# LordTARN1SHED/Image-Restoration-for-Road-Sign-Recognition-in-Autonomous-Driving

Hardware: AMD Instinct MI355X
Metric: images/sec ResUNet fwd+bwd (64x64 GTSRB batch) at 1/2/4/8 MI355X; PSNR parity (higher is better)
Workload: dtype bf16; 1 GPU; cfg3: ResUNet unified train step (dynamic distortion + ToTensor, fwd + L1 + 0.1*VGG16[:16] perceptual + bwd + AdamW), 14_train_unified_advanced.py; global_batch=512, per_gpu_batch=512, parallelism=dp1, hip_graph=True

## Files before the change

image-restoration-for-road-sign-recognition-in-autonomous-driving_amd/csrc/conv_in.hip:

```cpp
#include "common.h"

namespace {

template <typename T>
__global__ void conv_in_fwd_kernel(int n, int h, int w, int cin, int cout,
                                   const float *__restrict__ x, const float *__restrict__ wt,
                                   const float *__restrict__ b, int act, const float *alpha,
                                   T *__restrict__ y) {
  extern __shared__ __attribute__((aligned(16))) float sw[];
  const int kk = cin * 9;
  for (int i = threadIdx.x; i < kk * cout; i += blockDim.x) {
    const int co = i % cout, j = i / cout;
    sw[i] = wt[(long long)co * kk + j];
  }
  for (int i = threadIdx.x; i < cout; i += blockDim.x) sw[kk * cout + i] = b ? b[i] : 0.f;
  __syncthreads();
  const int G = cout / 4;
  const long long P = (long long)n * h * w;
  const float al = alpha ? alpha[0] : 0.f;
  for (long long id = blockIdx.x * (long long)blockDim.x + threadIdx.x; id < P * G;
       id += (long long)gridDim.x * blockDim.x) {
    const int g = (int)(id % G);
    const long long p = id / G;
    const int ww = (int)(p % w);
    const long long nh = p / w;
    const int hh = (int)(nh % h);
    const int nn = (int)(nh / h);
    f32x4 acc = *reinterpret_cast<const f32x4 *>(sw + kk * cout + g * 4);
    for (int ci = 0; ci < cin; ++ci) {
      const float *xp = x + ((long long)nn * cin + ci) * h * w;
#pragma unroll
      for (int t = 0; t < 9; ++t) {
        const int y2 = hh + t / 3 - 1, x2 = ww + t % 3 - 1;
        if (y2 < 0 || y2 >= h || x2 < 0 || x2 >= w) continue;
        const float v = xp[(long long)y2 * w + x2];
        acc += v * *reinterpret_cast<const f32x4 *>(sw + (ci * 9 + t) * cout + g * 4);
      }
    }
    if (act == 1) {
#pragma unroll
      for (int k = 0; k < 4; ++k) acc[k] = fmaxf(acc[k], 0.f);
    } else if (act == 2) {
#pragma unroll
      for (int k = 0; k < 4; ++k) acc[k] = acc[k] > 0.f ? acc[k] : al * acc[k];
    }
    store4<T>(y + p * cout + g * 4, acc);
  }
}

template <typename T>
__global__ void conv_in_wgrad_kernel(int n, int h, int w, int cin, int cout,
                                     const float *__restrict__ x, const T *__restrict__ dy,
                                     float *__restrict__ part, long long px_per_block) {
  __shared__ __attribute__((aligned(16))) float sdy[64][65];
  __shared__ __attribute__((aligned(16))) float spt[64][32];
  const int kk = cin * 9;
  const long long P = (long long)n * h * w;
  const long long pb = blockIdx.x * px_per_block;
  const long long pe = min(P, pb + px_per_block);
  const int co = threadIdx.x & 63, jg = threadIdx.x >> 6;
  double acc[8] = {0, 0, 0, 0, 0, 0, 0, 0};
  for (long long p0 = pb; p0 < pe; p0 += 64) {
    __syncthreads();
    for (int i = threadIdx.x; i < 64 * 64; i += blockDim.x) {
      const int r = i >> 6, c = i & 63;
      const long long p = p0 + r;
      sdy[r][c] = (p < pe && c < cout) ? Elt<T>::load(dy, p * cout + c) : 0.f;
    }
    for (int i = threadIdx.x; i < 64 * 32; i += blockDim.x) {
      const int r = i >> 5, j = i & 31;
      const long long p = p0 + r;
      float v = 0.f;
      if (p < pe) {
        if (j < kk) {
          const int ci = j / 9, t = j % 9;
          const int ww = (int)(p % w);
          const long long nh = p / w;
          const int hh = (int)(nh % h);
          const int nn = (int)(nh / h);
          const int y2 = hh + t / 3 - 1, x2 = ww + t % 3 - 1;
          if (y2 >= 0 && y2 < h && x2 >= 0 && x2 < w)
            v = x[(((long long)nn * cin + ci) * h + y2) * w + x2];
        } else if (j == kk) {
          v = 1.f;
        }
      }
      spt[r][j] = v;
    }
    __syncthreads();
    if (co < cout) {
      float st[8] = {0.f, 0.f, 0.f, 0.f, 0.f, 0.f, 0.f, 0.f};
#pragma unroll 4
      for (int r = 0; r < 64; ++r) {
        const float d = sdy[r][co];
        const f32x4 a0 = *reinterpret_cast<const f32x4 *>(&spt[r][jg * 8]);
        const f32x4 a1 = *reinterpret_cast<const f32x4 *>(&spt[r][jg * 8 + 4]);
#pragma unroll
        for (int k = 0; k < 4; ++k) { st[k] += d * a0[k]; st[4 + k] += d * a1[k]; }
      }
#pragma unroll
      for (int k = 0; k < 8; ++k) acc[k] += st[k];
    }
  }
  if (co < cout) {
#pragma unroll
    for (int k = 0; k < 8; ++k) part[((long long)blockIdx.x * cout + co) * 32 + jg * 8 + k] = (float)acc[k];
  }
}

constexpr int CIA_NPX = 64;
constexpr int CIA_ROW = CIA_NPX + 8;
constexpr int CIA_XROW = 32 + 8;
template <bool REC>
__global__ __launch_bounds__(256, REC ? 4 : 1) void conv_in_wgrad_act_kernel(
    int n, int h, int w, const float *__restrict__ x, const bf16_t *__restrict__ g,
    const bf16_t *__restrict__ t, int act, const float *__restrict__ alpha,
    float *__restrict__ part, long long ppb) {
  __shared__ __attribute__((aligned(16))) u16 gT[64 * CIA_ROW];
  __shared__ __attribute__((aligned(16))) u16 pT[32 * CIA_ROW];
  __shared__ __attribute__((aligned(16))) u16 pX[REC ? CIA_NPX * CIA_XROW : 8];
  __shared__ float red[256];
  const int tid = threadIdx.x, lane = tid & 63, wv = tid >> 6;
  const long long P = (long long)n * h * w, hw = (long long)h * w;
  const long long p0 = blockIdx.x * ppb, p1 = min(P, p0 + ppb);
  const float al = act == 2 ? alpha[0] : 0.f;
  float sa = 0.f;
  f32x4 acc[2] = {f32x4{0.f, 0.f, 0.f, 0.f}, f32x4{0.f, 0.f, 0.f, 0.f}};
  const int lc = tid & 7, lpp = tid >> 3;
  const int bn = lane & 15, bk = lane >> 4;
  const int sj = tid & 63, sg = tid >> 6;
  uint4 rg[2], rt[2] = {};
  float rp[8];
  auto load_step = [&](long long q0) __attribute__((always_inline)) {
#pragma unroll
    for (int j = 0; j < 2; ++j) {
      const long long p = q0 + 2 * lpp + j;
      const bool ok = p < p1;
      const long long e = (ok ? p : p0) * 64 + lc * 8;
      rg[j] = *reinterpret_cast<const uint4 *>(g + e);
      if constexpr (!REC) rt[j] = *reinterpret_cast<const uint4 *>(t + e);
      if (!ok) rg[j] = uint4{0u, 0u, 0u, 0u};
    }
    const long long p = q0 + sj;
    const bool live = p < p1;
    int img = 0, y = 0, xx0 = 0;
    if (live) {
      img = (int)(p / hw);
      const int rem = (int)(p - img * hw);
      y = rem / w;
      xx0 = rem - y * w;
    }
#pragma unroll
    for (int u = 0; u < 8; ++u) {
      const int r = sg + 4 * u;
      float val = 0.f;
      if (r < 27) {
        const int ci = r / 9, ky = (r % 9) / 3, kx = r % 3;
        const int yy = y + ky - 1, xx = xx0 + kx - 1;
        const bool ok = live && yy >= 0 && yy < h && xx >= 0 && xx < w;
        const float vv = x[ok ? (((long long)img * 3 + ci) * h + yy) * w + xx : 0];
        val = ok ? vv : 0.f;
      } else if (r == 27) {
        val = live ? 1.f : 0.f;
      }
      rp[u] = val;
    }
  };
  auto bf = [](uint32_t word, int hi) { return __uint_as_float(hi ? (word & 0xffff0000u) : (word << 16)); };
  bf16x8 fw = {};
  if constexpr (REC) fw = *reinterpret_cast<const bf16x8 *>(t + (wv * 16 + bn) * 32 + bk * 8);
  if (p0 < p1) load_step(p0);
  for (long long q0 = p0; q0 < p1; q0 += CIA_NPX) {
    if constexpr (REC) {
#pragma unroll
      for (int u = 0; u < 8; ++u) {
        const u16 pv = f32_to_bf16(rp[u]);
        pT[(sg + 4 * u) * CIA_ROW + sj] = pv;
        pX[sj * CIA_XROW + sg + 4 * u] = pv;
      }
      __syncthreads();
#pragma unroll
      for (int nb = 0; nb < 4; ++nb) {
        const bf16x8 fp = *reinterpret_cast<const bf16x8 *>(&pX[(nb * 16 + bn) * CIA_XROW + bk * 8]);
        const f32x4 tv = __builtin_amdgcn_mfma_f32_16x16x32_bf16(fw, fp, f32x4{0.f, 0.f, 0.f, 0.f}, 0, 0, 0);
#pragma unroll
        for (int i = 0; i < 4; ++i) gT[(wv * 16 + 4 * bk + i) * CIA_ROW + nb * 16 + bn] = f32_to_bf16(tv[i]);
      }
      __syncthreads();
    }
    u16 v[2][8];
    uint32_t tpair[8];
    if constexpr (REC) {
#pragma unroll
      for (int k = 0; k < 8; ++k)
        tpair[k] = *reinterpret_cast<const uint32_t *>(&gT[(lc * 8 + k) * CIA_ROW + 2 * lpp]);
    }
#pragma unroll
    for (int j = 0; j < 2; ++j) {
      const uint32_t gw[4] = {rg[j].x, rg[j].y, rg[j].z, rg[j].w};
      const uint32_t tw[4] = {rt[j].x, rt[j].y, rt[j].z, rt[j].w};
#pragma unroll
      for (int k = 0; k < 8; ++k) {
        const float gg = bf(gw[k >> 1], k & 1);
        const float tt = REC ? bf(tpair[k], j) : bf(tw[k >> 1], k & 1);
        const float gp = tt > 0.f ? gg : al * gg;
        sa += tt > 0.f ? 0.f : gg * tt;
        v[j][k] = f32_to_bf16(gp);
      }
    }
#pragma unroll
    for (int k = 0; k < 8; ++k)
      *reinterpret_cast<uint32_t *>(&gT[(lc * 8 + k) * CIA_ROW + 2 * lpp]) =
          (uint32_t)v[0][k] | ((uint32_t)v[1][k] << 16);
    if constexpr (!REC) {
#pragma unroll
      for (int u = 0; u < 8; ++u) pT[(sg + 4 * u) * CIA_ROW + sj] = f32_to_bf16(rp[u]);
    }
    __syncthreads();
    if (q0 + CIA_NPX < p1) load_step(q0 + CIA_NPX);
#pragma unroll
    for (int ks = 0; ks < 2; ++ks) {
      const int px = ks * 32 + bk * 8;
      const bf16x8 fa = *reinterpret_cast<const bf16x8 *>(&gT[(wv * 16 + bn) * CIA_ROW + px]);
#pragma unroll
      for (int nb = 0; nb < 2; ++nb) {
        const bf16x8 fb = *reinterpret_cast<const bf16x8 *>(&pT[(nb * 16 + bn) * CIA_ROW + px]);
        acc[nb] = __builtin_amdgcn_mfma_f32_16x16x32_bf16(fa, fb, acc[nb], 0, 0, 0);
      }
    }
    __syncthreads();
  }
  float *pw = part + (long long)blockIdx.x * (64 * 32 + 32);
#pragma unroll
  for (int nb = 0; nb < 2; ++nb)
#pragma unroll
    for (int i = 0; i < 4; ++i) pw[(wv * 16 + 4 * bk + i) * 32 + nb * 16 + bn] = acc[nb][i];
  red[tid] = sa;
  __syncthreads();
  for (int o = 128; o > 0; o >>= 1) {
    if (tid < o) red[tid] += red[tid + o];
    __syncthreads();
  }
  if (tid < 32) pw[64 * 32 + tid] = tid == 0 ? red[0] : 0.f;
}

__global__ void conv_in_wgrad_act_finalize(int chunks, const double *__restrict__ part, float *dw,
                                           float *db, float *dalpha) {
  const int i = blockIdx.x * blockDim.x + threadIdx.x;
  const int cols = 64 * 32 + 32;
  if (i > 64 * 32) return;
  double sv[1] = {0};
  rr_fixed_sum<1>(part + i, cols, chunks, sv);
  const double s = sv[0];
  if (i == 64 * 32) {
    if (dalpha) dalpha[0] = (float)s;
    return;
  }
  const int co = i / 32, j = i % 32;
  if (j < 27) dw[co * 27 + j] = (float)s;
  else if (j == 27 && db) db[co] = (float)s;
}

__global__ void conv_in_wgrad_finalize(int cout, int kk, int blocks, const double *__restrict__ part,
                                       float *dw, float *db) {
  const int i = blockIdx.x * blockDim.x + threadIdx.x;
  if (i >= cout * 32) return;
  const int co = i / 32, j = i % 32;
  if (j > kk) return;
  double sv[1] = {0};
  rr_fixed_sum<1>(part + i, (long long)cout * 32, blocks, sv);
  const double s = sv[0];
  if (j < kk) dw[(long long)co * kk + j] = (float)s;
  else if (db) db[co] = (float)s;
}

template <typename T>
__global__ void conv_in_dgrad_kernel(int n, int h, int w, int cin, int cout,
                                     const T *__restrict__ dy, const float *__restrict__ wt,
                                     float *__restrict__ dx, int accumulate) {
  extern __shared__ __attribute__((aligned(16))) float sw[];
  const int kk = cin * 9;
  for (int i = threadIdx.x; i < kk * cout; i += blockDim.x) {
    const int co = i % cout, j = i / cout;
    const int t = j / cin, ci = j % cin;
    sw[i] = wt[((long long)co * cin + ci) * 9 + t];
  }
  __syncthreads();
  const long long P = (long long)n * h * w;
  for (long long p = blockIdx.x * (long long)blockDim.x + threadIdx.x; p < P;
       p += (long long)gridDim.x * blockDim.x) {
    const int ww = (int)(p % w);
    const long long nh = p / w;
    const int hh = (int)(nh % h);
    const int nn = (int)(nh / h);
    float acc[4] = {0.f, 0.f, 0.f, 0.f};
    for (int t = 0; t < 9; ++t) {
      const int ky = t / 3, kx = t % 3;
      const int y2 = hh - ky + 1, x2 = ww - kx + 1;
      if (y2 < 0 || y2 >= h || x2 < 0 || x2 >= w) continue;
      const T *dp = dy + (((long long)nn * h + y2) * w + x2) * cout;
      for (int c = 0; c < cout; c += 4) {
        const f32x4 d = load4<T>(dp + c);
        for (int ci = 0; ci < cin && ci < 4; ++ci) {
          const f32x4 wv = *reinterpret_cast<const f32x4 *>(sw + (t * cin + ci) * cout + c);
          acc[ci] += d[0] * wv[0] + d[1] * wv[1] + d[2] * wv[2] + d[3] * wv[3];
        }
      }
    }
    for (int ci = 0; ci < cin && ci < 4; ++ci) {
      const long long o = (((long long)nn * cin + ci) * h + hh) * w + ww;
      dx[o] = accumulate ? dx[o] + acc[ci] : acc[ci];
    }
  }
}

template <typename T>
__global__ void im2col3_kernel(int n, int h, int w, int cin, int kpad, const float *__restrict__ x,
                               T *__restrict__ col) {
  const int G = kpad / 4;
  const long long total = (long long)n * h * w * G;
  const int kk = cin * 9;
  for (long long i = blockIdx.x * (long long)blockDim.x + threadIdx.x; i < total;
       i += (long long)gridDim.x * blockDim.x) {
    const int g = (int)(i % G);
    const long long p = i / G;
    const int ww = (int)(p % w);
    const long long nh = p / w;
    const int hh = (int)(nh % h);
    const int nn = (int)(nh / h);
    f32x4 v;
#pragma unroll
    for (int e = 0; e < 4; ++e) {
      const int j = g * 4 + e;
      float val = 0.f;
      if (j < kk) {
        const int ci = j / 9, t = j - (j / 9) * 9;
        const int y2 = hh + t / 3 - 1, x2 = ww + t % 3 - 1;
        if (y2 >= 0 && y2 < h && x2 >= 0 && x2 < w)
          val = x[(((long long)nn * cin + ci) * h + y2) * w + x2];
      } else if (j == kk) {
        val = 1.f;
      }
      v[e] = val;
    }
    store4<T>(col + p * kpad + g * 4, v);
  }
}

__global__ __launch_bounds__(256) void conv_in_mfma_kernel(int n, int h, int w,
                                                           const float *__restrict__ x,
                                                           const bf16_t *__restrict__ wp, int act,
                                                           const float *__restrict__ alpha,
                                                           bf16_t *__restrict__ y_pre,
                                                           bf16_t *__restrict__ y_act) {
  constexpr int SR = 68;
  __shared__ __attribute__((aligned(16))) float stg[4][32 * SR];
  const int lane = threadIdx.x & 63, wv = threadIdx.x >> 6;
  const long long hw = (long long)h * w;
  const long long P = (long long)n * hw;
  const long long p0 = ((long long)blockIdx.x * 4 + wv) * 64;
  if (p0 >= P) return;
  const int fr = lane & 15, q = lane >> 4;
  bf16x8 fa[4];
#pragma unroll
  for (int mi = 0; mi < 4; ++mi)
    fa[mi] = *reinterpret_cast<const bf16x8 *>(wp + (mi * 16 + fr) * 32 + q * 8);
  const int hwi = h * w;
  int kofs[8], kdy[8], kdx[8];
  bool ktap[8], kone[8];
#pragma unroll
  for (int j = 0; j < 8; ++j) {
    const int k = q * 8 + j;
    const int ci = k / 9, t = k - (k / 9) * 9;
    kdy[j] = t / 3 - 1;
    kdx[j] = t % 3 - 1;
    kofs[j] = ci * hwi + kdy[j] * w + kdx[j];
    ktap[j] = k < 27;
    kone[j] = k == 27;
  }
  const int Pi = (int)P;
  const __amdgpu_buffer_rsrc_t xr = __builtin_amdgcn_make_buffer_rsrc(
      const_cast<float *>(x), 0, (int)(3 * P * 4), 0x00020000);
  const int pw0 = (int)p0;
  f32x4 acc[4][4];
#pragma unroll
  for (int ni = 0; ni < 4; ++ni) {
    const int p = pw0 + ni * 16 + fr;
    const bool live = p < Pi;
    const int pc = live ? p : 0;
    const int nn = pc / hwi, rem = pc - (pc / hwi) * hwi;
    const int yy = rem / w, xx = rem - (rem / w) * w;
    const int base = nn * 3 * hwi + rem;
    bf16x8 fb;
#pragma unroll
    for (int j = 0; j < 8; ++j) {
      const int y2 = yy + kdy[j], x2 = xx + kdx[j];
      const bool ok = ktap[j] && live && (unsigned)y2 < (unsigned)h && (unsigned)x2 < (unsigned)w;
      const float v = __builtin_bit_cast(float, __builtin_amdgcn_raw_buffer_load_b32(
          xr, ok ? (base + kofs[j]) * 4 : 0xffffffff, 0, 0));
      fb[j] = (__bf16)(v + (kone[j] ? 1.f : 0.f));
    }
#pragma unroll
    for (int mi = 0; mi < 4; ++mi)
      acc[mi][ni] = __builtin_amdgcn_mfma_f32_16x16x32_bf16(fa[mi], fb, f32x4{0.f, 0.f, 0.f, 0.f},
                                                           0, 0, 0);
  }
  float *sw = stg[wv];
  const float slope = act == 2 ? alpha[0] : (act == 1 ? 0.f : 1.f);
  const int rows = (int)min(64LL, P - p0);
#pragma unroll
  for (int half = 0; half < 2; ++half) {
    if (half) asm volatile("s_waitcnt lgkmcnt(0)" ::: "memory");
#pragma unroll
    for (int mi = 0; mi < 4; ++mi)
#pragma unroll
      for (int nj = 0; nj < 2; ++nj)
        *reinterpret_cast<f32x4 *>(sw + (nj * 16 + fr) * SR + mi * 16 + q * 4) = acc[mi][half * 2 + nj];
    asm volatile("s_waitcnt lgkmcnt(0)" ::: "memory");
#pragma unroll
    for (int i = 0; i < 4; ++i) {
      const int rl = i * 8 + (lane >> 3), c8 = (lane & 7) * 8;
      const int r = half * 32 + rl;
      if (r < rows) {
        const long long p = p0 + r;
        const f32x4 v0 = *reinterpret_cast<const f32x4 *>(sw + rl * SR + c8);
        const f32x4 v1 = *reinterpret_cast<const f32x4 *>(sw + rl * SR + c8 + 4);
        if (y_pre) store8<bf16_t>(y_pre + p * 64 + c8, v0, v1);
        if (y_act) {
          f32x4 a0, a1;
#pragma unroll
          for (int k = 0; k < 4; ++k) {
            a0[k] = v0[k] > 0.f ? v0[k] : slope * v0[k];
            a1[k] = v1[k] > 0.f ? v1[k] : slope * v1[k];
          }
          store8<bf16_t>(y_act + p * 64 + c8, a0, a1);
        }
      }
    }
  }
}

}

extern "C" int rr_im2col3(int dtype, int n, int h, int w, int cin, int kpad, const float *x,
                          void *col, rr_stream stream) {
  if (!x || !col || cin <= 0 || kpad % 4 || kpad < 9 * cin + 1) return RR_EINVAL;
  const long long total = (long long)n * h * w * (kpad / 4);
  dim3 g(rr_grid_cap((total + 255) / 256, 8192)), b(256);
  hipStream_t st = (hipStream_t)stream;
  return rr_dispatch_elt(dtype, [&](auto tag) {
    using T = typename decltype(tag)::type;
    hipLaunchKernelGGL(im2col3_kernel<T>, g, b, 0, st, n, h, w, cin, kpad, x, (T *)col);
    RR_CHECK_LAUNCH();
    return RR_OK;
  });
}

extern "C" int rr_conv_in_fwd(int dtype, int n, int h, int w, int cin, int cout, const float *x,
                              const float *wt, const float *b, int act, const float *alpha,
                              void *y, rr_stream stream) {
  if (!x || !wt || !y || n <= 0 || h <= 0 || w <= 0 || cin <= 0 || cin > 4 || cout % 4 ||
      cout > 128 || (act == 2 && !alpha))
    return RR_EINVAL;
  const long long work = (long long)n * h * w * (cout / 4);
  const size_t shm = ((size_t)cin * 9 * cout + cout) * sizeof(float);
  dim3 g(rr_grid_cap((work + 255) / 256, 8192)), bl(256);
  hipStream_t st = (hipStream_t)stream;
  return rr_dispatch_elt(dtype, [&](auto tag) {
    using T = typename decltype(tag)::type;
    hipLaunchKernelGGL(conv_in_fwd_kernel<T>, g, bl, shm, st, n, h, w, cin, cout, x, wt, b, act,
                       alpha, (T *)y);
    RR_CHECK_LAUNCH();
    return RR_OK;
  });
}

int rr_colreduce_misc(const float *in, int rows, int cols, double *out, hipStream_t st);
static int conv_in_wgrad_blocks(int n, int h, int w) {
  const long long P = (long long)n * h * w;
  long long b = (P + 2047) / 2048;
  if (b > 1024) b = 1024;
  return (int)(b < 1 ? 1 : b);
}

extern "C" size_t rr_conv_in_wgrad_workspace(int n, int h, int w, int cin, int cout) {
  (void)cin;
  const int blocks = conv_in_wgrad_blocks(n, h, w);
  return (size_t)blocks * cout * 32 * sizeof(float) + rr_colreduce_bytes(blocks, cout * 32);
}

extern "C" int rr_conv_in_wgrad(int dtype, int n, int h, int w, int cin, int cout, const float *x,
                                const void *dy, float *dw, float *db, void *ws, size_t ws_bytes,
                                rr_stream stream) {
  if (!x || !dy || !dw || cin * 9 >= 32 || cout > 64 || cout <= 0) return RR_EINVAL;
  const int blocks = conv_in_wgrad_blocks(n, h, w);
  const size_t pbytes = (size_t)blocks * cout * 32 * sizeof(float);
  if (!ws || ws_bytes < pbytes + rr_colreduce_bytes(blocks, cout * 32)) return RR_EWORKSPACE;
  const long long P = (long long)n * h * w;
  long long ppb = (P + blocks - 1) / blocks;
  hipStream_t st = (hipStream_t)stream;
  const int rc = rr_dispatch_elt(dtype, [&](auto tag) {
    using T = typename decltype(tag)::type;
    hipLaunchKernelGGL(conv_in_wgrad_kernel<T>, dim3(blocks), dim3(256), 0, st, n, h, w, cin, cout,
                       x, (const T *)dy, (float *)ws, ppb);
    RR_CHECK_LAUNCH();
    return RR_OK;
  });
  if (rc != RR_OK) return rc;
  double *red = (double *)((char *)ws + pbytes);
  const int chunks = rr_colreduce_misc((const float *)ws, blocks, cout * 32, red, st);
  if (chunks < 0) return RR_ELAUNCH;
  hipLaunchKernelGGL(conv_in_wgrad_finalize, dim3((cout * 32 + 255) / 256), dim3(256), 0, st, cout,
                     cin * 9, chunks, (const double *)red, dw, db);
  RR_CHECK_LAUNCH();
  return RR_OK;
}

static int conv_in_act_blocks(long long P) {
  long long b = (P + 511) / 512;
  if (b > 2048) b = 2048;
  return (int)(b < 1 ? 1 : b);
}

extern "C" size_t rr_conv_in_wgrad_act_workspace(int n, int h, int w) {
  const int blocks = conv_in_act_blocks((long long)n * h * w);
  return (size_t)blocks * (64 * 32 + 32) * sizeof(float) + rr_colreduce_bytes(blocks, 64 * 32 + 32);
}

static int conv_in_wgrad_act(bool rec, int n, int h, int w, const float *x, const void *dy,
                             const void *t_pre, int act, const float *alpha, float *dw, float *db,
                             float *dalpha, void *ws, size_t ws_bytes, rr_stream stream) {
  if (!x || !dy || !t_pre || !dw || n <= 0 || h <= 0 || w <= 0) return RR_EINVAL;
  if (act < 1 || act > 2 || (act == 2 && !alpha)) return RR_EINVAL;
// ... 67 lines not shown
```

image-restoration-for-road-sign-recognition-in-autonomous-driving_amd/csrc/conv_out.hip:

```cpp
#include "common.h"

namespace {

template <typename T>
__global__ void conv_out_fwd_kernel(int n, int h, int w, int cin, int cout, const T *__restrict__ x,
                                    const float *__restrict__ wt, const float *__restrict__ b,
                                    float *__restrict__ y) {
  extern __shared__ __attribute__((aligned(16))) float sw[];
  for (int i = threadIdx.x; i < cin * cout; i += blockDim.x) sw[i] = wt[i];
  __syncthreads();
  const long long P = (long long)n * h * w;
  const long long hw = (long long)h * w;
  for (long long p = blockIdx.x * (long long)blockDim.x + threadIdx.x; p < P;
       p += (long long)gridDim.x * blockDim.x) {
    float acc[4] = {0.f, 0.f, 0.f, 0.f};
    const T *xp = x + p * cin;
    for (int c = 0; c < cin; c += 4) {
      const f32x4 v = load4<T>(xp + c);
      for (int co = 0; co < cout && co < 4; ++co) {
        const f32x4 wv = *reinterpret_cast<const f32x4 *>(sw + co * cin + c);
        acc[co] += v[0] * wv[0] + v[1] * wv[1] + v[2] * wv[2] + v[3] * wv[3];
      }
    }
    const long long nn = p / hw, r = p % hw;
    for (int co = 0; co < cout && co < 4; ++co)
      y[(nn * cout + co) * hw + r] = acc[co] + (b ? b[co] : 0.f);
  }
}

template <typename T>
__global__ void conv_out_bwd_kernel(int n, int h, int w, int cin, int cout,
                                    const float *__restrict__ dy, const T *__restrict__ x,
                                    const float *__restrict__ wt, T *__restrict__ dx, int mask_relu,
                                    float *__restrict__ part, long long px_per_block) {
  __shared__ float red[4][64][4];
  __shared__ float redb[4][4];
  const int ci = threadIdx.x & 63, row = threadIdx.x >> 6;
  const long long hw = (long long)h * w;
  const long long P = (long long)n * hw;
  const long long pb = blockIdx.x * px_per_block;
  const long long pe = min(P, pb + px_per_block);
  float wv[4] = {0.f, 0.f, 0.f, 0.f};
  for (int co = 0; co < cout; ++co) wv[co] = ci < cin ? wt[co * cin + ci] : 0.f;
  float sw[4] = {0.f, 0.f, 0.f, 0.f}, sb[4] = {0.f, 0.f, 0.f, 0.f};
  for (long long p = pb + row; p < pe; p += 4) {
    const long long nn = p / hw, r = p - nn * hw;
    float d[4] = {0.f, 0.f, 0.f, 0.f};
    for (int co = 0; co < cout; ++co) d[co] = dy[(nn * cout + co) * hw + r];
    if (ci < cin) {
      const float xv = Elt<T>::load(x, p * cin + ci);
      float g = 0.f;
      for (int co = 0; co < cout; ++co) {
        g += d[co] * wv[co];
        sw[co] += d[co] * xv;
      }
      if (mask_relu && !(xv > 0.f)) g = 0.f;
      if (dx) Elt<T>::store(dx, p * cin + ci, g);
    }
    for (int co = 0; co < cout; ++co) sb[co] += d[co];
  }
  for (int co = 0; co < 4; ++co) red[row][ci][co] = sw[co];
  if (ci == 0)
    for (int co = 0; co < 4; ++co) redb[row][co] = sb[co];
  __syncthreads();
  if (row == 0 && ci < cin)
    for (int co = 0; co < cout; ++co)
      part[((long long)blockIdx.x * (cout + 1) + co) * cin + ci] =
          red[0][ci][co] + red[1][ci][co] + red[2][ci][co] + red[3][ci][co];
  if (threadIdx.x < cout) {
    const int co = threadIdx.x;
    part[((long long)blockIdx.x * (cout + 1) + cout) * cin + co] =
        redb[0][co] + redb[1][co] + redb[2][co] + redb[3][co];
  }
}

template <typename T, int COUT>
__global__ __launch_bounds__(256) void conv_out_bwd64_kernel(
    int n, int h, int w, const float *__restrict__ dy, const T *__restrict__ x,
    const float *__restrict__ wt, T *__restrict__ dx, int mask_relu, float *__restrict__ part,
    long long px_per_block) {
  constexpr int CIN = 64;
  __shared__ float red[4][COUT + 1][CIN];
  const int cg = threadIdx.x & 7, pl = threadIdx.x >> 3;
  const long long hw = (long long)h * w;
  const long long P = (long long)n * hw;
  const long long pb = blockIdx.x * px_per_block;
  const long long pe = min(P, pb + px_per_block);
  float wv[COUT][8];
#pragma unroll
  for (int co = 0; co < COUT; ++co)
#pragma unroll
    for (int j = 0; j < 8; ++j) wv[co][j] = wt[co * CIN + cg * 8 + j];
  float sw[COUT][8], sb[COUT];
#pragma unroll
  for (int co = 0; co < COUT; ++co) {
    sb[co] = 0.f;
#pragma unroll
    for (int j = 0; j < 8; ++j) sw[co][j] = 0.f;
  }
  auto one = [&](long long p) __attribute__((always_inline)) {
    const long long nn = p / hw, r = p - nn * hw;
    float d[COUT];
#pragma unroll
    for (int co = 0; co < COUT; ++co) d[co] = dy[(nn * COUT + co) * hw + r];
    const T *xp = x + p * CIN + cg * 8;
    const f32x4 x0 = load4<T>(xp), x1 = load4<T>(xp + 4);
    const float xv[8] = {x0[0], x0[1], x0[2], x0[3], x1[0], x1[1], x1[2], x1[3]};
    float g[8];
#pragma unroll
    for (int j = 0; j < 8; ++j) {
      float t = 0.f;
#pragma unroll
      for (int co = 0; co < COUT; ++co) {
        t += d[co] * wv[co][j];
        sw[co][j] += d[co] * xv[j];
      }
      g[j] = (mask_relu && !(xv[j] > 0.f)) ? 0.f : t;
    }
#pragma unroll
    for (int co = 0; co < COUT; ++co) sb[co] += d[co];
    if (dx) store8<T>(dx + p * CIN + cg * 8, f32x4{g[0], g[1], g[2], g[3]}, f32x4{g[4], g[5], g[6], g[7]});
  };
  long long p = pb + pl;
  for (; p + 32 < pe; p += 64) {
    one(p);
    one(p + 32);
  }
  if (p < pe) one(p);
#pragma unroll
  for (int co = 0; co < COUT; ++co) {
#pragma unroll
    for (int j = 0; j < 8; ++j) {
      float v = sw[co][j];
      v += __shfl_xor(v, 8, 64);
      v += __shfl_xor(v, 16, 64);
      v += __shfl_xor(v, 32, 64);
      sw[co][j] = v;
    }
    float v = sb[co];
    v += __shfl_xor(v, 8, 64);
    v += __shfl_xor(v, 16, 64);
    v += __shfl_xor(v, 32, 64);
    sb[co] = v;
  }
  const int wv_ = threadIdx.x >> 6, lane = threadIdx.x & 63;
  if (lane < 8) {
#pragma unroll
    for (int co = 0; co < COUT; ++co) {
#pragma unroll
      for (int j = 0; j < 8; ++j) red[wv_][co][cg * 8 + j] = sw[co][j];
      if (cg == 0) red[wv_][COUT][co] = sb[co];
    }
  }
  __syncthreads();
  for (int i = threadIdx.x; i < COUT * CIN + COUT; i += 256) {
    const int co = i / CIN, ci = i - co * CIN;
    part[(long long)blockIdx.x * (COUT + 1) * CIN + i] =
        red[0][co][ci] + red[1][co][ci] + red[2][co][ci] + red[3][co][ci];
  }
}

template <typename T, int COUT, bool REC = false>
__global__ __launch_bounds__(256) void conv_out_bwd64_bnred_kernel(
    int n, int h, int w, const float *__restrict__ dy, const T *__restrict__ x,
    const float *__restrict__ wt, const T *__restrict__ t0, const float *__restrict__ mean0,
    const float *__restrict__ inv0, const T *__restrict__ t1, const float *__restrict__ mean1,
    const float *__restrict__ inv1, float *__restrict__ part, float *__restrict__ bnpart,
    long long px_per_block, const float *__restrict__ aff_s = nullptr,
    const float *__restrict__ aff_b = nullptr) {
  constexpr int CIN = 64;
  __shared__ float red[4][COUT + 1][CIN];
  __shared__ float bred[4][CIN][3];
  const int cg = threadIdx.x & 7, pl = threadIdx.x >> 3;
  const long long hw = (long long)h * w;
  const long long P = (long long)n * hw;
  const long long pb = blockIdx.x * px_per_block;
  const long long pe = min(P, pb + px_per_block);
  float wv[COUT][8], m0[8], i0[8], m1[8], i1[8];
#pragma unroll
  for (int j = 0; j < 8; ++j) {
#pragma unroll
    for (int co = 0; co < COUT; ++co) wv[co][j] = wt[co * CIN + cg * 8 + j];
    m0[j] = mean0[cg * 8 + j]; i0[j] = inv0[cg * 8 + j];
    m1[j] = mean1[cg * 8 + j]; i1[j] = inv1[cg * 8 + j];
  }
  __shared__ __attribute__((aligned(16))) float faff[REC ? 4 * CIN : 4];
  if constexpr (REC) {
    faff[threadIdx.x] = threadIdx.x < 2 * CIN ? aff_s[threadIdx.x] : aff_b[threadIdx.x - 2 * CIN];
    __syncthreads();
  }
  float sw[COUT][8], sb[COUT], bs[3][8];
#pragma unroll
  for (int co = 0; co < COUT; ++co) {
    sb[co] = 0.f;
#pragma unroll
    for (int j = 0; j < 8; ++j) sw[co][j] = 0.f;
  }
#pragma unroll
  for (int j = 0; j < 8; ++j) { bs[0][j] = 0.f; bs[1][j] = 0.f; bs[2][j] = 0.f; }
  auto one = [&](long long p) __attribute__((always_inline)) {
    const long long nn = p / hw, r = p - nn * hw;
    float d[COUT];
#pragma unroll
    for (int co = 0; co < COUT; ++co) d[co] = dy[(nn * COUT + co) * hw + r];
    const long long e = p * CIN + cg * 8;
    f32x4 x0, x1, a0, a1, b0, b1;
    load8<T>(t0 + e, a0, a1);
    load8<T>(t1 + e, b0, b1);
    if constexpr (REC) {
      int o = cg * 8;
      asm volatile("" : "+v"(o));
      const f32x4 *fa = reinterpret_cast<const f32x4 *>(faff + o);
      f32x4 v0 = a0 * fa[0] + fa[32], v1 = a1 * fa[1] + fa[33];
      f32x4 q0 = b0 * fa[16] + fa[48], q1 = b1 * fa[17] + fa[49];
      v0 += q0;
      v1 += q1;
#pragma unroll
      for (int k = 0; k < 4; ++k) {
        x0[k] = Elt<T>::round(fmaxf(v0[k], 0.f));
        x1[k] = Elt<T>::round(fmaxf(v1[k], 0.f));
      }
    } else {
      load8<T>(x + e, x0, x1);
    }
    const float xv[8] = {x0[0], x0[1], x0[2], x0[3], x1[0], x1[1], x1[2], x1[3]};
    const float ta[8] = {a0[0], a0[1], a0[2], a0[3], a1[0], a1[1], a1[2], a1[3]};
    const float tb[8] = {b0[0], b0[1], b0[2], b0[3], b1[0], b1[1], b1[2], b1[3]};
#pragma unroll
    for (int j = 0; j < 8; ++j) {
      float t = 0.f;
#pragma unroll
      for (int co = 0; co < COUT; ++co) {
        t += d[co] * wv[co][j];
        sw[co][j] += d[co] * xv[j];
      }
      const float gm = xv[j] > 0.f ? Elt<T>::round(t) : 0.f;
      bs[0][j] += gm;
      bs[1][j] += gm * ((ta[j] - m0[j]) * i0[j]);
      bs[2][j] += gm * ((tb[j] - m1[j]) * i1[j]);
    }
#pragma unroll
    for (int co = 0; co < COUT; ++co) sb[co] += d[co];
  };
  long long p = pb + pl;
  for (; p + 32 < pe; p += 64) {
    one(p);
    one(p + 32);
  }
  if (p < pe) one(p);
  auto lanes8 = [](float v) __attribute__((always_inline)) {
    v += __shfl_xor(v, 8, 64);
    v += __shfl_xor(v, 16, 64);
    v += __shfl_xor(v, 32, 64);
    return v;
  };
#pragma unroll
  for (int co = 0; co < COUT; ++co) {
#pragma unroll
    for (int j = 0; j < 8; ++j) sw[co][j] = lanes8(sw[co][j]);
    sb[co] = lanes8(sb[co]);
  }
#pragma unroll
  for (int k = 0; k < 3; ++k)
#pragma unroll
    for (int j = 0; j < 8; ++j) bs[k][j] = lanes8(bs[k][j]);
  const int wv_ = threadIdx.x >> 6, lane = threadIdx.x & 63;
  if (lane < 8) {
#pragma unroll
    for (int co = 0; co < COUT; ++co) {
#pragma unroll
      for (int j = 0; j < 8; ++j) red[wv_][co][cg * 8 + j] = sw[co][j];
      if (cg == 0) red[wv_][COUT][co] = sb[co];
    }
#pragma unroll
    for (int j = 0; j < 8; ++j)
#pragma unroll
      for (int k = 0; k < 3; ++k) bred[wv_][cg * 8 + j][k] = bs[k][j];
  }
  __syncthreads();
  for (int i = threadIdx.x; i < COUT * CIN + COUT; i += 256) {
    const int co = i / CIN, ci = i - co * CIN;
    part[(long long)blockIdx.x * (COUT + 1) * CIN + i] =
        red[0][co][ci] + red[1][co][ci] + red[2][co][ci] + red[3][co][ci];
  }
  if (threadIdx.x < CIN * 3) {
    const int c = threadIdx.x / 3, k = threadIdx.x - c * 3;
    bnpart[(long long)blockIdx.x * CIN * 3 + threadIdx.x] =
        bred[0][c][k] + bred[1][c][k] + bred[2][c][k] + bred[3][c][k];
  }
}

constexpr int TCO_D = 2;
__global__ __launch_bounds__(256) void tail_conv_out_kernel(
    int P, int hw, int cout, const bf16_t *__restrict__ x, const float *__restrict__ scale,
    const float *__restrict__ shift, const bf16_t *__restrict__ res, const float *__restrict__ rs,
    const float *__restrict__ rb, const bf16_t *__restrict__ wp, const float *__restrict__ bias,
    bf16_t *__restrict__ y, float *__restrict__ out) {
  const int lane = threadIdx.x & 63;
  const int wv = __builtin_amdgcn_readfirstlane(threadIdx.x >> 6);
  const int fr = lane & 15, fq = lane >> 4;
  const int nblk = (P + 15) >> 4;
  const int gw = blockIdx.x * 4 + wv, NWT = gridDim.x * 4;
  bf16x8 wr[2];
  f32x4 s[2][2], b[2][2], qs[2][2], qb[2][2];
#pragma unroll
  for (int kb = 0; kb < 2; ++kb) {
    bf16x8 v = {};
    if (fr < cout) v = *reinterpret_cast<const bf16x8 *>(wp + fr * 64 + kb * 32 + fq * 8);
    wr[kb] = v;
#pragma unroll
    for (int hf = 0; hf < 2; ++hf) {
      const int c = kb * 32 + fq * 8 + 4 * hf;
      s[kb][hf] = *reinterpret_cast<const f32x4 *>(scale + c);
      b[kb][hf] = *reinterpret_cast<const f32x4 *>(shift + c);
      qs[kb][hf] = *reinterpret_cast<const f32x4 *>(rs + c);
      qb[kb][hf] = *reinterpret_cast<const f32x4 *>(rb + c);
    }
  }
  float bv[4];
#pragma unroll
  for (int j = 0; j < 4; ++j) bv[j] = j < cout ? bias[j] : 0.f;
  struct Blk {
    uint4 t[2], r[2];
  };
  auto load_blk = [&](int bi, Blk &bk) __attribute__((always_inline)) {
    const int p = min(bi * 16 + fr, P - 1);
    const long long e = (long long)p * 64 + fq * 8;
#pragma unroll
    for (int kb = 0; kb < 2; ++kb) {
      bk.t[kb] = *reinterpret_cast<const uint4 *>(x + e + kb * 32);
      bk.r[kb] = *reinterpret_cast<const uint4 *>(res + e + kb * 32);
    }
  };
  auto unpack = [](uint4 r, f32x4 &lo, f32x4 &hi) __attribute__((always_inline)) {
    lo[0] = __uint_as_float(r.x << 16); lo[1] = __uint_as_float(r.x & 0xffff0000u);
    lo[2] = __uint_as_float(r.y << 16); lo[3] = __uint_as_float(r.y & 0xffff0000u);
    hi[0] = __uint_as_float(r.z << 16); hi[1] = __uint_as_float(r.z & 0xffff0000u);
    hi[2] = __uint_as_float(r.w << 16); hi[3] = __uint_as_float(r.w & 0xffff0000u);
  };
  auto run = [&](const Blk &bk, int bi) __attribute__((always_inline)) {
    const int p = bi * 16 + fr;
    const bool live = p < P;
    f32x4 acc = f32x4{0.f, 0.f, 0.f, 0.f};
#pragma unroll
    for (int kb = 0; kb < 2; ++kb) {
      f32x4 v0, v1, q0, q1;
      unpack(bk.t[kb], v0, v1);
      unpack(bk.r[kb], q0, q1);
      v0 = v0 * s[kb][0] + b[kb][0];
      v1 = v1 * s[kb][1] + b[kb][1];
      q0 = q0 * qs[kb][0] + qb[kb][0];
      q1 = q1 * qs[kb][1] + qb[kb][1];
      v0 += q0;
      v1 += q1;
#pragma unroll
      for (int k = 0; k < 4; ++k) { v0[k] = fmaxf(v0[k], 0.f); v1[k] = fmaxf(v1[k], 0.f); }
      u16x8 r;
      r[0] = f32_to_bf16(v0[0]); r[1] = f32_to_bf16(v0[1]); r[2] = f32_to_bf16(v0[2]); r[3] = f32_to_bf16(v0[3]);
      r[4] = f32_to_bf16(v1[0]); r[5] = f32_to_bf16(v1[1]); r[6] = f32_to_bf16(v1[2]); r[7] = f32_to_bf16(v1[3]);
      if (y && live) *reinterpret_cast<u16x8 *>(y + (long long)p * 64 + kb * 32 + fq * 8) = r;
      acc = __builtin_amdgcn_mfma_f32_16x16x32_bf16(wr[kb], __builtin_bit_cast(bf16x8, r), acc, 0, 0, 0);
    }
    if (live && fq == 0) {
      const int n = p / hw, rem = p - n * hw;
#pragma unroll
      for (int j = 0; j < 4; ++j)
        if (j < cout) out[((long long)n * cout + j) * hw + rem] = acc[j] + bv[j];
    }
  };
  for (int b0 = gw; b0 < nblk; b0 += TCO_D * NWT) {
    Blk bk[TCO_D];
#pragma unroll
    for (int j = 0; j < TCO_D; ++j) load_blk(min(b0 + j * NWT, nblk - 1), bk[j]);
#pragma unroll
    for (int j = 0; j < TCO_D; ++j)
      if (b0 + j * NWT < nblk) run(bk[j], b0 + j * NWT);
  }
}

__global__ void conv_out_bwd_finalize(int cin, int cout, int blocks, const double *__restrict__ part,
                                      float *dw, float *db) {
  const int i = blockIdx.x * blockDim.x + threadIdx.x;
  if (i >= cout * cin + cout) return;
  double s = 0;
  if (i < cout * cin) {
    double sv[1] = {0};
    rr_fixed_sum<1>(part + i, (long long)(cout + 1) * cin, blocks, sv);
    s = sv[0];
    if (dw) dw[i] = (float)s;
  } else {
    const int co = i - cout * cin;
    double sv[1] = {0};
    rr_fixed_sum<1>(part + (long long)cout * cin + co, (long long)(cout + 1) * cin, blocks, sv);
    s = sv[0];
    if (db) db[co] = (float)s;
  }
}

}

extern "C" int rr_conv_out_fwd(int dtype, int n, int h, int w, int cin, int cout, const void *x,
                               const float *wt, const float *b, float *y, rr_stream stream) {
  if (!x || !wt || !y || cout > 4 || cout <= 0 || cin % 4) return RR_EINVAL;
  const long long P = (long long)n * h * w;
  dim3 g(rr_grid_cap((P + 255) / 256, 8192)), bl(256);
  const size_t shm = (size_t)cin * cout * sizeof(float);
  hipStream_t st = (hipStream_t)stream;
  return rr_dispatch_elt(dtype, [&](auto tag) {
    using T = typename decltype(tag)::type;
    hipLaunchKernelGGL(conv_out_fwd_kernel<T>, g, bl, shm, st, n, h, w, cin, cout, (const T *)x, wt,
                       b, y);
    RR_CHECK_LAUNCH();
    return RR_OK;
  });
}

int rr_colreduce_misc(const float *in, int rows, int cols, double *out, hipStream_t st);
static int conv_out_blocks(int n, int h, int w) {
  const long long P = (long long)n * h * w;
  long long b = (P + 1023) / 1024;
  if (b > 2048) b = 2048;
  return (int)(b < 1 ? 1 : b);
}

extern "C" size_t rr_conv_out_bwd_workspace(int n, int h, int w, int cin, int cout) {
  const int blocks = conv_out_blocks(n, h, w);
  return (size_t)blocks * (cout + 1) * cin * sizeof(float) +
         rr_colreduce_bytes(blocks, (cout + 1) * cin);
}

extern "C" int rr_conv_out_bwd(int dtype, int n, int h, int w, int cin, int cout, const float *dy,
                               const void *x, const float *wt, void *dx, int mask_relu, float *dw,
                               float *db, void *ws, size_t ws_bytes, rr_stream stream) {
  if (!dy || !x || !wt || cout > 4 || cout <= 0 || cin > 64 || cin < cout) return RR_EINVAL;
  const int blocks = conv_out_blocks(n, h, w);
  const size_t pbytes = (size_t)blocks * (cout + 1) * cin * sizeof(float);
  if (!ws || ws_bytes < pbytes + rr_colreduce_bytes(blocks, (cout + 1) * cin)) return RR_EWORKSPACE;
  const long long P = (long long)n * h * w;
  const long long ppb = (P + blocks - 1) / blocks;
  hipStream_t st = (hipStream_t)stream;
  const int rc = cin == 64 && cout == 3 ? rr_dispatch_elt(dtype, [&](auto tag) {
    using T = typename decltype(tag)::type;
    hipLaunchKernelGGL((conv_out_bwd64_kernel<T, 3>), dim3(blocks), dim3(256), 0, st, n, h, w, dy,
                       (const T *)x, wt, (T *)dx, mask_relu, (float *)ws, ppb);
    RR_CHECK_LAUNCH();
    return RR_OK;
  }) : rr_dispatch_elt(dtype, [&](auto tag) {
    using T = typename decltype(tag)::type;
    hipLaunchKernelGGL(conv_out_bwd_kernel<T>, dim3(blocks), dim3(256), 0, st, n, h, w, cin, cout, dy,
                       (const T *)x, wt, (T *)dx, mask_relu, (float *)ws, ppb);
    RR_CHECK_LAUNCH();
    return RR_OK;
  });
  if (rc != RR_OK) return rc;
  double *red = (double *)((char *)ws + pbytes);
  const int chunks = rr_colreduce_misc((const float *)ws, blocks, (cout + 1) * cin, red, st);
  if (chunks < 0) return RR_ELAUNCH;
  hipLaunchKernelGGL(conv_out_bwd_finalize, dim3((cout * cin + cout + 255) / 256), dim3(256), 0,
                     st, cin, cout, chunks, (const double *)red, dw, db);
  RR_CHECK_LAUNCH();
  return RR_OK;
}

extern "C" size_t rr_conv_out_bwd_bnred_workspace(long long P, int cin, int cout) {
  const int blocks = rr_bn_stats_blocks(P);
  return (size_t)blocks * (cout + 1) * cin * sizeof(float) + rr_colreduce_bytes(blocks, (cout + 1) * cin);
}

static int conv_out_bwd_bnred(const rr_bnbwd_desc *d, int n, int h, int w, int cout, const float *dy,
                              const void *x, const float *aff_s, const float *aff_b, const float *wt,
                              const void *t0, const float *mean0, const float *invstd0, const void *t1,
                              const float *mean1, const float *invstd1, float *dw, float *db,
                              float *bn_partial, void *ws, size_t ws_bytes, rr_stream stream) {
  const bool rec = x == nullptr;
  if (!d || !dy || !wt || !t0 || !mean0 || !invstd0 || !t1 || !mean1 || !invstd1 || !dw || !db ||
      !bn_partial || (rec && (!aff_s || !aff_b)))
    return RR_EINVAL;
  const long long P = (long long)n * h * w;
  if (d->P != P || d->nbn != 2 || d->mask_kind != 4 || d->eval) return RR_EINVAL;
  if (rec && !rr_dtype_ok(d->dtype)) return RR_EINVAL;
  if (d->C != 64 || cout != 3 || (rec && d->dtype != RR_BF16)) return RR_EUNSUPPORTED;
  const int blocks = rr_bn_stats_blocks(P);
  if (blocks != rr_bn_bwd_blocks(d)) return RR_EINVAL;
  const size_t pbytes = (size_t)blocks * (cout + 1) * d->C * sizeof(float);
  if (!ws || ws_bytes < rr_conv_out_bwd_bnred_workspace(P, d->C, cout)) return RR_EWORKSPACE;
  const long long ppb = (P + blocks - 1) / blocks;
  hipStream_t st = (hipStream_t)stream;
  int rc;
  if (rec) {
    using T = bf16_t;
    hipLaunchKernelGGL((conv_out_bwd64_bnred_kernel<T, 3, true>), dim3(blocks), dim3(256), 0, st, n, h, w,
                       dy, (const T *)nullptr, wt, (const T *)t0, mean0, invstd0, (const T *)t1, mean1,
                       invstd1, (float *)ws, bn_partial, ppb, aff_s, aff_b);
    RR_CHECK_LAUNCH();
    rc = RR_OK;
  } else {
    rc = rr_dispatch_elt(d->dtype, [&](auto tag) {
      using T = typename decltype(tag)::type;
      hipLaunchKernelGGL((conv_out_bwd64_bnred_kernel<T, 3>), dim3(blocks), dim3(256), 0, st, n, h, w, dy,
                         (const T *)x, wt, (const T *)t0, mean0, invstd0, (const T *)t1, mean1, invstd1,
                         (float *)ws, bn_partial, ppb, (const float *)nullptr, (const float *)nullptr);
      RR_CHECK_LAUNCH();
      return RR_OK;
    });
  }
  if (rc != RR_OK) return rc;
  double *red = (double *)((char *)ws + pbytes);
  const int chunks = rr_colreduce_misc((const float *)ws, blocks, (cout + 1) * d->C, red, st);
  if (chunks < 0) return RR_ELAUNCH;
  hipLaunchKernelGGL(conv_out_bwd_finalize, dim3((cout * d->C + cout + 255) / 256), dim3(256), 0, st, d->C,
                     cout, chunks, (const double *)red, dw, db);
  RR_CHECK_LAUNCH();
  return RR_OK;
}

extern "C" int rr_conv_out_bwd_bnred(const rr_bnbwd_desc *d, int n, int h, int w, int cout,
                                     const float *dy, const void *x, const float *wt, const void *t0,
                                     const float *mean0, const float *invstd0, const void *t1,
                                     const float *mean1, const float *invstd1, float *dw, float *db,
                                     float *bn_partial, void *ws, size_t ws_bytes, rr_stream stream) {
  if (!x) return RR_EINVAL;
  return conv_out_bwd_bnred(d, n, h, w, cout, dy, x, nullptr, nullptr, wt, t0, mean0, invstd0, t1, mean1,
                            invstd1, dw, db, bn_partial, ws, ws_bytes, stream);
}

extern "C" int rr_conv_out_bwd_bnred_rec(int n, int h, int w, int cout, const rr_bnbwd_desc *d,
                                         const float *dy, const float *wt, const float *aff_s,
                                         const float *aff_b, const void *t0, const float *mean0,
                                         const float *invstd0, const void *t1, const float *mean1,
                                         const float *invstd1, float *dw, float *db, float *bn_partial,
                                         void *ws, size_t ws_bytes, rr_stream stream) {
  return conv_out_bwd_bnred(d, n, h, w, cout, dy, nullptr, aff_s, aff_b, wt, t0, mean0, invstd0, t1,
                            mean1, invstd1, dw, db, bn_partial, ws, ws_bytes, stream);
}

extern "C" int rr_affine_act_conv_out(int x_dtype, int n, int h, int w, int C, int cout, const void *x,
                                      const float *scale, const float *shift, const void *res,
                                      const float *res_scale, const float *res_shift,
                                      const void *wpack, const float *bias, void *y, float *out,
                                      rr_stream stream) {
  if (!rr_dtype_ok(x_dtype) || n <= 0 || h <= 0 || w <= 0 || C <= 0 || cout <= 0 || !x || !scale ||
      !shift || !res || !res_scale || !res_shift || !wpack || !bias || !out)
    return RR_EINVAL;
  const long long P = (long long)n * h * w;
  if (x_dtype != RR_BF16 || C != 64 || cout > 4 || P > 0x7fffffffLL - 16) return RR_EUNSUPPORTED;
  const int nblk = (int)((P + 15) / 16);
  const int grid = rr_grid_cap(((long long)nblk + 4 * TCO_D - 1) / (4 * TCO_D), 2048);
// ... 8 lines not shown
```

Baseline: 36300 images/sec.

## Double-buffer input-conv wgrad with swizzled LDS and transpose reads; strength-reduce indexing

Reworks the first-layer conv weight-gradient kernel. It now double-buffers the gradient and patch tiles in LDS with XOR-swizzled layouts and reads the MFMA fragments with ds_read_tr16 transposing loads. In the recompute path the MFMA for the previous tile overlaps the production of the next one, which removes a barrier per step. Patch gathering now uses precomputed tap offsets and incremental pixel coordinates instead of per-step divisions. In the output-conv backward kernel, the affine coefficients move from shared memory into registers and the dy index is stepped incrementally; the cost is more registers and more complex buffer bookkeeping.

After: 36340 images/sec (median of 3 runs). About the same (+0.1%).

```diff
diff --git a/image-restoration-for-road-sign-recognition-in-autonomous-driving_amd/csrc/conv_in.hip b/image-restoration-for-road-sign-recognition-in-autonomous-driving_amd/csrc/conv_in.hip
--- a/image-restoration-for-road-sign-recognition-in-autonomous-driving_amd/csrc/conv_in.hip
+++ b/image-restoration-for-road-sign-recognition-in-autonomous-driving_amd/csrc/conv_in.hip
@@ -109,18 +109,33 @@
 }
 
 constexpr int CIA_NPX = 64;
-constexpr int CIA_ROW = CIA_NPX + 8;
-constexpr int CIA_XROW = 32 + 8;
+constexpr int CIA_GROW = 128;
+constexpr int CIA_PROW = 64;
+constexpr int CIA_TROW = 144;
+__device__ __forceinline__ int cia_gswz(int p) { return 2 * ((0x10323210u >> (4 * ((p >> 1) & 7))) & 0xf); }
+__device__ __forceinline__ int cia_pswz(int p) { return (p >> 2) & 2; }
+
+typedef short cia_s16x8 __attribute__((ext_vector_type(8)));
+__device__ __forceinline__ bf16x8 cia_tr_frag(const char *p0, const char *p1) {
+  const s16x4 lo = __builtin_amdgcn_ds_read_tr16_b64_v4i16(
+      (__attribute__((address_space(3))) s16x4 *)LDS_PTR(p0));
+  const s16x4 hi = __builtin_amdgcn_ds_read_tr16_b64_v4i16(
+      (__attribute__((address_space(3))) s16x4 *)LDS_PTR(p1));
+  const cia_s16x8 v = __builtin_shufflevector(lo, hi, 0, 1, 2, 3, 4, 5, 6, 7);
+  return __builtin_bit_cast(bf16x8, v);
+}
+
 template <bool REC>
 __global__ __launch_bounds__(256, REC ? 4 : 1) void conv_in_wgrad_act_kernel(
     int n, int h, int w, const float *__restrict__ x, const bf16_t *__restrict__ g,
     const bf16_t *__restrict__ t, int act, const float *__restrict__ alpha,
     float *__restrict__ part, long long ppb) {
-  __shared__ __attribute__((aligned(16))) u16 gT[64 * CIA_ROW];
-  __shared__ __attribute__((aligned(16))) u16 pT[32 * CIA_ROW];
-  __shared__ __attribute__((aligned(16))) u16 pX[REC ? CIA_NPX * CIA_XROW : 8];
+  __shared__ __attribute__((aligned(16))) char sG[2][CIA_NPX * CIA_GROW];
+  __shared__ __attribute__((aligned(16))) char sP[2][CIA_NPX * CIA_PROW];
+  __shared__ __attribute__((aligned(16))) char sT[REC ? CIA_NPX * CIA_TROW : 16];
   __shared__ float red[256];
-  const int tid = threadIdx.x, lane = tid & 63, wv = tid >> 6;
+  const int tid = threadIdx.x, lane = tid & 63;
+  const int wv = __builtin_amdgcn_readfirstlane(tid >> 6);
   const long long P = (long long)n * h * w, hw = (long long)h * w;
   const long long p0 = blockIdx.x * ppb, p1 = min(P, p0 + ppb);
   const float al = act == 2 ? alpha[0] : 0.f;
@@ -128,10 +143,27 @@
   f32x4 acc[2] = {f32x4{0.f, 0.f, 0.f, 0.f}, f32x4{0.f, 0.f, 0.f, 0.f}};
   const int lc = tid & 7, lpp = tid >> 3;
   const int bn = lane & 15, bk = lane >> 4;
-  const int sj = tid & 63, sg = tid >> 6;
+  const int sj = lane, sg = wv;
+  long long kofs[8];
+  int ktap[8];
+#pragma unroll
+  for (int u = 0; u < 8; ++u) {
+    const int r = 8 * sg + u, ci = r / 9;
+    ktap[u] = r - 9 * ci;
+    kofs[u] = ci * hw + (ktap[u] / 3 - 1) * w + (ktap[u] % 3 - 1);
+  }
+  int gy, gx;
+  long long gb;
+  {
+    const long long p = p0 + sj, img = p / hw;
+    const int rem = (int)(p - img * hw);
+    gy = rem / w;
+    gx = rem - gy * w;
+    gb = img * 3 * hw + rem;
+  }
   uint4 rg[2], rt[2] = {};
   float rp[8];
-  auto load_step = [&](long long q0) __attribute__((always_inline)) {
+  auto load_g = [&](long long q0) __attribute__((always_inline)) {
 #pragma unroll
     for (int j = 0; j < 2; ++j) {
       const long long p = q0 + 2 * lpp + j;
@@ -141,94 +173,128 @@
       if constexpr (!REC) rt[j] = *reinterpret_cast<const uint4 *>(t + e);
       if (!ok) rg[j] = uint4{0u, 0u, 0u, 0u};
     }
-    const long long p = q0 + sj;
-    const bool live = p < p1;
-    int img = 0, y = 0, xx0 = 0;
-    if (live) {
-      img = (int)(p / hw);
-      const int rem = (int)(p - img * hw);
-      y = rem / w;
-      xx0 = rem - y * w;
-    }
+  };
+  auto load_patch = [&](long long q0) __attribute__((always_inline)) {
+    const bool live = q0 + sj < p1;
+    const int xm = (gx > 0 ? 1 : 0) | 2 | (gx < w - 1 ? 4 : 0);
+    const int inside = !live ? 0 : (gy > 0 ? xm : 0) | (xm << 3) | (gy < h - 1 ? xm << 6 : 0);
 #pragma unroll
     for (int u = 0; u < 8; ++u) {
-      const int r = sg + 4 * u;
+      const int r = 8 * sg + u;
       float val = 0.f;
       if (r < 27) {
-        const int ci = r / 9, ky = (r % 9) / 3, kx = r % 3;
-        const int yy = y + ky - 1, xx = xx0 + kx - 1;
-        const bool ok = live && yy >= 0 && yy < h && xx >= 0 && xx < w;
-        const float vv = x[ok ? (((long long)img * 3 + ci) * h + yy) * w + xx : 0];
+        const bool ok = (inside >> ktap[u]) & 1;
+        const float vv = x[ok ? gb + kofs[u] : 0];
         val = ok ? vv : 0.f;
       } else if (r == 27) {
         val = live ? 1.f : 0.f;
       }
       rp[u] = val;
+    }
+    gx += CIA_NPX;
+    gb += CIA_NPX;
+    while (gx >= w) {
+      gx -= w;
+      ++gy;
+    }
+    while (gy >= h) {
+      gy -= h;
+      gb += 2 * hw;
     }
   };
   auto bf = [](uint32_t word, int hi) { return __uint_as_float(hi ? (word & 0xffff0000u) : (word << 16)); };
   bf16x8 fw = {};
   if constexpr (REC) fw = *reinterpret_cast<const bf16x8 *>(t + (wv * 16 + bn) * 32 + bk * 8);
-  if (p0 < p1) load_step(p0);
-  for (long long q0 = p0; q0 < p1; q0 += CIA_NPX) {
-    if constexpr (REC) {
-#pragma unroll
-      for (int u = 0; u < 8; ++u) {
-        const u16 pv = f32_to_bf16(rp[u]);
-        pT[(sg + 4 * u) * CIA_ROW + sj] = pv;
-        pX[sj * CIA_XROW + sg + 4 * u] = pv;
-      }
-      __syncthreads();
-#pragma unroll
-      for (int nb = 0; nb < 4; ++nb) {
-        const bf16x8 fp = *reinterpret_cast<const bf16x8 *>(&pX[(nb * 16 + bn) * CIA_XROW + bk * 8]);
-        const f32x4 tv = __builtin_amdgcn_mfma_f32_16x16x32_bf16(fw, fp, f32x4{0.f, 0.f, 0.f, 0.f}, 0, 0, 0);
-#pragma unroll
-        for (int i = 0; i < 4; ++i) gT[(wv * 16 + 4 * bk + i) * CIA_ROW + nb * 16 + bn] = f32_to_bf16(tv[i]);
-      }
-      __syncthreads();
-    }
-    u16 v[2][8];
-    uint32_t tpair[8];
-    if constexpr (REC) {
-#pragma unroll
-      for (int k = 0; k < 8; ++k)
-        tpair[k] = *reinterpret_cast<const uint32_t *>(&gT[(lc * 8 + k) * CIA_ROW + 2 * lpp]);
-    }
+  int ao[2], bo[2][2];
+  {
+    const int q = (lane >> 2) & 3, pp = lane & 3;
+#pragma unroll
+    for (int hf = 0; hf < 2; ++hf) {
+      const int p = 8 * bk + 4 * hf + q;
+      ao[hf] = p * CIA_GROW + (((2 * wv + (pp >> 1)) ^ cia_gswz(p)) << 4) + 8 * (pp & 1);
+#pragma unroll
+      for (int nb = 0; nb < 2; ++nb)
+        bo[nb][hf] = p * CIA_PROW + (((2 * nb + (pp >> 1)) ^ cia_pswz(p)) << 4) + 8 * (pp & 1);
+    }
+  }
+  auto wgrad_mfma = [&](int b) __attribute__((always_inline)) {
+#pragma unroll
+    for (int ks = 0; ks < 2; ++ks) {
+      const char *ga = sG[b] + ks * 32 * CIA_GROW, *pa = sP[b] + ks * 32 * CIA_PROW;
+      const bf16x8 fa = cia_tr_frag(ga + ao[0], ga + ao[1]);
+#pragma unroll
+      for (int nb = 0; nb < 2; ++nb) {
+        const bf16x8 fb = cia_tr_frag(pa + bo[nb][0], pa + bo[nb][1]);
+        acc[nb] = __builtin_amdgcn_mfma_f32_16x16x32_bf16(fa, fb, acc[nb], 0, 0, 0);
+      }
+    }
+  };
+  auto store_patch = [&](int b) __attribute__((always_inline)) {
+    u16x8 pv;
+#pragma unroll
+    for (int u = 0; u < 8; ++u) pv[u] = f32_to_bf16(rp[u]);
+    *reinterpret_cast<u16x8 *>(sP[b] + sj * CIA_PROW + ((sg ^ cia_pswz(sj)) << 4)) = pv;
+  };
+  auto store_gp = [&](int b) __attribute__((always_inline)) {
 #pragma unroll
     for (int j = 0; j < 2; ++j) {
       const uint32_t gw[4] = {rg[j].x, rg[j].y, rg[j].z, rg[j].w};
       const uint32_t tw[4] = {rt[j].x, rt[j].y, rt[j].z, rt[j].w};
+      u16x8 v;
 #pragma unroll
       for (int k = 0; k < 8; ++k) {
         const float gg = bf(gw[k >> 1], k & 1);
-        const float tt = REC ? bf(tpair[k], j) : bf(tw[k >> 1], k & 1);
+        const float tt = bf(tw[k >> 1], k & 1);
         const float gp = tt > 0.f ? gg : al * gg;
         sa += tt > 0.f ? 0.f : gg * tt;
-        v[j][k] = f32_to_bf16(gp);
-      }
-    }
-#pragma unroll
-    for (int k = 0; k < 8; ++k)
-      *reinterpret_cast<uint32_t *>(&gT[(lc * 8 + k) * CIA_ROW + 2 * lpp]) =
-          (uint32_t)v[0][k] | ((uint32_t)v[1][k] << 16);
+        v[k] = f32_to_bf16(gp);
+      }
+      const int p = 2 * lpp + j;
+      *reinterpret_cast<u16x8 *>(sG[b] + p * CIA_GROW + ((lc ^ cia_gswz(p)) << 4)) = v;
+    }
+  };
+  if (p0 < p1) {
+    load_g(p0);
+    load_patch(p0);
+  }
+  int b = 0;
+  for (long long q0 = p0; q0 < p1; q0 += CIA_NPX, b ^= 1) {
+    const bool more = q0 + CIA_NPX < p1;
+    store_patch(b);
     if constexpr (!REC) {
-#pragma unroll
-      for (int u = 0; u < 8; ++u) pT[(sg + 4 * u) * CIA_ROW + sj] = f32_to_bf16(rp[u]);
-    }
-    __syncthreads();
-    if (q0 + CIA_NPX < p1) load_step(q0 + CIA_NPX);
-#pragma unroll
-    for (int ks = 0; ks < 2; ++ks) {
-      const int px = ks * 32 + bk * 8;
-      const bf16x8 fa = *reinterpret_cast<const bf16x8 *>(&gT[(wv * 16 + bn) * CIA_ROW + px]);
-#pragma unroll
-      for (int nb = 0; nb < 2; ++nb) {
-        const bf16x8 fb = *reinterpret_cast<const bf16x8 *>(&pT[(nb * 16 + bn) * CIA_ROW + px]);
-        acc[nb] = __builtin_amdgcn_mfma_f32_16x16x32_bf16(fa, fb, acc[nb], 0, 0, 0);
-      }
-    }
-    __syncthreads();
+      store_gp(b);
+      __syncthreads();
+      if (more) {
+        load_g(q0 + CIA_NPX);
+        load_patch(q0 + CIA_NPX);
+      }
+      wgrad_mfma(b);
+    } else {
+      if (more) load_patch(q0 + CIA_NPX);
+      __syncthreads();
+#pragma unroll
+      for (int nb = 0; nb < 4; ++nb) {
+        const int p = nb * 16 + bn;
+        const bf16x8 fp = *reinterpret_cast<const bf16x8 *>(sP[b] + p * CIA_PROW + ((bk ^ cia_pswz(p)) << 4));
+        const f32x4 tv = __builtin_amdgcn_mfma_f32_16x16x32_bf16(fw, fp, f32x4{0.f, 0.f, 0.f, 0.f}, 0, 0, 0);
+        uint2 tw;
+        tw.x = (uint32_t)f32_to_bf16(tv[0]) | ((uint32_t)f32_to_bf16(tv[1]) << 16);
+        tw.y = (uint32_t)f32_to_bf16(tv[2]) | ((uint32_t)f32_to_bf16(tv[3]) << 16);
+        *reinterpret_cast<uint2 *>(sT + p * CIA_TROW + (wv * 16 + 4 * bk) * 2) = tw;
+      }
+      if (q0 != p0) wgrad_mfma(b ^ 1);
+      __syncthreads();
+#pragma unroll
+      for (int j = 0; j < 2; ++j) rt[j] = *reinterpret_cast<const uint4 *>(sT + (2 * lpp + j) * CIA_TROW + lc * 16);
+      store_gp(b);
+      if (more) load_g(q0 + CIA_NPX);
+    }
+  }
+  if constexpr (REC) {
+    if (p0 < p1) {
+      __syncthreads();
+      wgrad_mfma(b ^ 1);
+    }
   }
   float *pw = part + (long long)blockIdx.x * (64 * 32 + 32);
 #pragma unroll
diff --git a/image-restoration-for-road-sign-recognition-in-autonomous-driving_amd/csrc/conv_out.hip b/image-restoration-for-road-sign-recognition-in-autonomous-driving_amd/csrc/conv_out.hip
--- a/image-restoration-for-road-sign-recognition-in-autonomous-driving_amd/csrc/conv_out.hip
+++ b/image-restoration-for-road-sign-recognition-in-autonomous-driving_amd/csrc/conv_out.hip
@@ -184,10 +184,15 @@
     m0[j] = mean0[cg * 8 + j]; i0[j] = inv0[cg * 8 + j];
     m1[j] = mean1[cg * 8 + j]; i1[j] = inv1[cg * 8 + j];
   }
-  __shared__ __attribute__((aligned(16))) float faff[REC ? 4 * CIN : 4];
+  f32x4 fs[2][2] = {}, fb[2][2] = {};
   if constexpr (REC) {
-    faff[threadIdx.x] = threadIdx.x < 2 * CIN ? aff_s[threadIdx.x] : aff_b[threadIdx.x - 2 * CIN];
-    __syncthreads();
+#pragma unroll
+    for (int k = 0; k < 2; ++k)
+#pragma unroll
+      for (int hf = 0; hf < 2; ++hf) {
+        fs[k][hf] = *reinterpret_cast<const f32x4 *>(aff_s + k * CIN + cg * 8 + 4 * hf);
+        fb[k][hf] = *reinterpret_cast<const f32x4 *>(aff_b + k * CIN + cg * 8 + 4 * hf);
+      }
   }
   float sw[COUT][8], sb[COUT], bs[3][8];
 #pragma unroll
@@ -198,21 +203,25 @@
   }
 #pragma unroll
   for (int j = 0; j < 8; ++j) { bs[0][j] = 0.f; bs[1][j] = 0.f; bs[2][j] = 0.f; }
+  long long p = pb + pl;
+  long long r = p % hw, dyo = (p / hw) * COUT * hw + r;
   auto one = [&](long long p) __attribute__((always_inline)) {
-    const long long nn = p / hw, r = p - nn * hw;
     float d[COUT];
 #pragma unroll
-    for (int co = 0; co < COUT; ++co) d[co] = dy[(nn * COUT + co) * hw + r];
+    for (int co = 0; co < COUT; ++co) d[co] = dy[dyo + co * hw];
+    r += 32;
+    dyo += 32;
+    while (r >= hw) {
+      r -= hw;
+      dyo += (COUT - 1) * hw;
+    }
     const long long e = p * CIN + cg * 8;
     f32x4 x0, x1, a0, a1, b0, b1;
     load8<T>(t0 + e, a0, a1);
     load8<T>(t1 + e, b0, b1);
     if constexpr (REC) {
-      int o = cg * 8;
-      asm volatile("" : "+v"(o));
-      const f32x4 *fa = reinterpret_cast<const f32x4 *>(faff + o);
-      f32x4 v0 = a0 * fa[0] + fa[32], v1 = a1 * fa[1] + fa[33];
-      f32x4 q0 = b0 * fa[16] + fa[48], q1 = b1 * fa[17] + fa[49];
+      f32x4 v0 = a0 * fs[0][0] + fb[0][0], v1 = a1 * fs[0][1] + fb[0][1];
+      f32x4 q0 = b0 * fs[1][0] + fb[1][0], q1 = b1 * fs[1][1] + fb[1][1];
       v0 += q0;
       v1 += q1;
 #pragma unroll
@@ -242,7 +251,6 @@
 #pragma unroll
     for (int co = 0; co < COUT; ++co) sb[co] += d[co];
   };
-  long long p = pb + pl;
   for (; p + 32 < pe; p += 64) {
     one(p);
     one(p + 32);
```
